# yixuan/LBFGSpp

Measured on AMD Instinct MI355X. Metric: L-BFGS iterations/sec at n=10^8, m=10; achieved HBM GB/s vs peak, higher is better.
Workload: dtype f64; 1 GPU; north-star: extended Rosenbrock n=100000000 m=10 f64 LineSearchMoreThuente, x0 from counter hash; n=100000000, m=10, history_full=True, fevals_total=111, apply_Hv_persistent_launches=82

## Files before the change

### include/lbfgsx.h

```cpp
#ifndef LBFGSX_H
#define LBFGSX_H

#include <stddef.h>
#include <stdint.h>

#ifdef __cplusplus
extern "C" {
#endif

typedef struct lbfgsx_ctx lbfgsx_ctx;

enum { LBFGSX_F64 = 0, LBFGSX_F32 = 1 };
enum { LBFGSX_OBJ_NONE = -1, LBFGSX_OBJ_DIAG_QUAD = 0, LBFGSX_OBJ_EXT_ROSENBROCK = 1,
       LBFGSX_OBJ_BOUND = 64  };
enum
{
    LBFGSX_OK = 0,
    LBFGSX_E_INVALID = -1,
    LBFGSX_E_LOGIC = -2,
    LBFGSX_E_RUNTIME = -3,
    LBFGSX_E_HIP = -4,
    LBFGSX_E_NOGPU = -5,
    LBFGSX_E_USER = -6
};
// ... 49 lines not shown
int lbfgsx_trial(lbfgsx_ctx* c, int objective, double step, double* fx, double* dg);
int lbfgsx_trial_point(lbfgsx_ctx* c, double step);
int lbfgsx_trial_dg(lbfgsx_ctx* c, double* dg);
int lbfgsx_ls_keep_trial_as_lo(lbfgsx_ctx* c);
int lbfgsx_ls_end(lbfgsx_ctx* c, int use_lo);
int lbfgsx_post_linesearch(lbfgsx_ctx* c, double* gnorm2, double* xnorm2, double* sy, double* yy);
int lbfgsx_commit_correction(lbfgsx_ctx* c);
int lbfgsx_post_linesearch_spec(lbfgsx_ctx* c, double a, double* gnorm2, double* xnorm2, double* sy, double* yy);
int lbfgsx_spec_counts(const lbfgsx_ctx* c, int64_t out[3]);
int lbfgsx_ls_post_in_trial(lbfgsx_ctx* c, double a);
int lbfgsx_post_in_trial_counts(const lbfgsx_ctx* c, int64_t out[4]);
int lbfgsx_last_in_trial_request(lbfgsx_ctx* c, int on);
int lbfgsx_apply_Hv_pending(lbfgsx_ctx* c, int v_which, double a, double* dg, int* pending);
int lbfgsx_trial_first(lbfgsx_ctx* c, int objective, double step, double* fx, double* dg, double* dg_init);
int lbfgsx_last_in_trial_counts(const lbfgsx_ctx* c, int64_t out[4]);
typedef struct lbfgsx_objective lbfgsx_objective;
int lbfgsx_objective_compile(lbfgsx_objective** out, int dtype, int K, const char* body, char* log, size_t log_len);
void lbfgsx_objective_destroy(lbfgsx_objective* obj);
long long lbfgsx_objective_source(int dtype, int K, const char* body, char* out, size_t len);
int lbfgsx_objective_info(const lbfgsx_objective* obj, long long out[8]);
int lbfgsx_objective_K(const lbfgsx_objective* obj);
int lbfgsx_objective_dtype(const lbfgsx_objective* obj);
int lbfgsx_objective_bind(lbfgsx_ctx* c, const lbfgsx_objective* obj, const void* const p[4], const double cs[8], int* id);
int lbfgsx_objective_upload(lbfgsx_ctx* c, int slot, const void* host, void** dev);
int lbfgsx_objective_bound(const lbfgsx_ctx* c, const void* p[4]);
enum { LBFGSX_FORM_TERM = 0, LBFGSX_FORM_CHAIN = 1, LBFGSX_FORM_GRID = 2, LBFGSX_FORM_GRAPH = 3, LBFGSX_FORM_MESH = 4, LBFGSX_FORM_LINEAR = 5,
       LBFGSX_FORM_LINEAR_MULTI = 6, LBFGSX_FORM_DENSE = 7, LBFGSX_FORM_LINEAR_GRAPH = 8, LBFGSX_FORM_VOLUME = 9,
       LBFGSX_FORM_GRID_PERIODIC = 10, LBFGSX_FORM_VOLUME_PERIODIC = 11, LBFGSX_FORM_GRID_FIELD = 12,
       LBFGSX_FORM_GRID_STENCIL = 13 };
int lbfgsx_objective_compile_chain(lbfgsx_objective** out, int dtype, int K, const char* body, char* log, size_t log_len);
// ... 282 lines not shown
```

### lbfgspp_amd/_lib.py

```python
import ctypes as C
import os

HERE = os.path.dirname(os.path.abspath(__file__))

F64, F32 = 0, 1
OBJ_DIAG_QUAD, OBJ_EXT_ROSENBROCK = 0, 1
OBJ_BOUND = 64
LS_NOCEDAL_WRIGHT, LS_MORE_THUENTE, LS_BACKTRACKING, LS_BRACKETING = 0, 1, 2, 3
ALGO_LBFGS, ALGO_LBFGSB = 0, 1
RECURSION_VECTOR, RECURSION_GRAM_SPACE, RECURSION_GRAM_SPACE_F32H = 0, 1, 2
FLAG_BOUNDED = 1
(VEC_X, VEC_G, VEC_XP, VEC_GP, VEC_D, VEC_XT, VEC_GT, VEC_A, VEC_B, VEC_LB, VEC_UB, VEC_XCP) = range(12)
E_INVALID, E_LOGIC, E_RUNTIME, E_HIP, E_NOGPU, E_USER = -1, -2, -3, -4, -5, -6


class Params(C.Structure):
    _fields_ = [("m", C.c_int), ("epsilon", C.c_double), ("epsilon_rel", C.c_double), ("past", C.c_int),
                ("delta", C.c_double), ("max_iterations", C.c_int), ("linesearch", C.c_int),
                ("max_linesearch", C.c_int), ("min_step", C.c_double), ("max_step", C.c_double),
                ("ftol", C.c_double), ("wolfe", C.c_double), ("max_submin", C.c_int)]


class Result(C.Structure):
    _fields_ = [("niter", C.c_int), ("nfev", C.c_int), ("fx", C.c_double), ("gnorm", C.c_double),
# ... 86 lines not shown
    sig(core, "lbfgsx_timing_enable", i32, vp, i32)
    sig(core, "lbfgsx_timing_read", i32, vp, pd, C.POINTER(i64), pd, C.POINTER(i64))
    sig(core, "lbfgsx_stream_probe", i32, vp, i32, pd, pd)
    sig(core, "lbfgsx_selftest_reduce", i32, vp, i32, i32, i32, pd)
    sig(core, "lbfgsx_post_linesearch_spec", i32, vp, dbl, pd, pd, pd, pd)
    sig(core, "lbfgsx_rccl_allgather_records", i32, C.POINTER(i32), i32, vp, i64, i64, C.POINTER(vp))
    sig(core, "lbfgsx_device_download", i32, i32, vp, i64, vp)
    sig(core, "lbfgsx_device_free", None, i32, vp)
    sig(core, "lbfgsx_spec_counts", i32, vp, C.POINTER(i64 * 3))
    sig(core, "lbfgsx_ls_post_in_trial", i32, vp, dbl)
    sig(core, "lbfgsx_post_in_trial_counts", i32, vp, C.POINTER(i64 * 4))
    sig(core, "lbfgsx_last_in_trial_request", i32, vp, i32)
    sig(core, "lbfgsx_apply_Hv_pending", i32, vp, i32, dbl, pd, C.POINTER(i32))
    sig(core, "lbfgsx_trial_first", i32, vp, i32, dbl, pd, pd, pd)
    sig(core, "lbfgsx_last_in_trial_counts", i32, vp, C.POINTER(i64 * 4))
    sig(core, "lbfgsx_counters", i32, C.POINTER(i64 * 3), i32)
    sig(core, "lbfgsx_counters_ex", i32, C.POINTER(i64 * 8), i32)
    sig(core, "lbfgsx_poll_counts", i32, vp, C.POINTER(i64 * 2))
    sig(core, "lbfgsx_poll_counts_ex", i32, vp, C.POINTER(i64 * 4))
    sig(core, "lbfgsx_b_compact_vec_counts", i32, C.POINTER(i64 * 4), i32)
    sig(core, "lbfgsx_b_reserve", i32, vp)
    sig(core, "lbfgsx_device", i32, vp)
    sig(core, "lbfgsx_persist_counts", i32, vp, C.POINTER(i64 * 4))
    sig(core, "lbfgsx_debug_persist_fault", i32, vp)

    sig(sol, "lbfgsx_solver_create", i32, C.POINTER(vp), i32, i32, i32, C.POINTER(Params), i32)
    sig(sol, "lbfgsx_solver_create_error", C.c_char_p)
    sig(sol, "lbfgsx_solver_destroy", None, vp)
    sig(sol, "lbfgsx_solver_prepare", i32, vp, i64)
    sig(sol, "lbfgsx_solver_ctx", vp, vp)
# ... 186 lines not shown
```

### lbfgspp_amd/csrc/ctx.hpp

```cpp
#pragma once
#include <hip/hip_runtime.h>
#include <stdint.h>

#include <atomic>
#include <chrono>
#include <string>
#include <vector>

#include "../../include/lbfgsx.h"
#include "last_step.hpp"
#include "reduce.cuh"

struct lbfgsx_ctx;
namespace lbfgsx {

void set_error(const std::string& msg);

#define LBFGSX_HIP(expr)                                                                      \
    do                                                                                        \
    {                                                                                         \
        hipError_t e_ = (expr);                                                               \
        if (e_ != hipSuccess)                                                                 \
        {                                                                                     \
            lbfgsx::set_error(std::string(#expr) + ": " + hipGetErrorString(e_) + " [" + __FILE__ + ":" + std::to_string(__LINE__) + "]");            \
            return LBFGSX_E_HIP;                                                              \
// ... 177 lines not shown
    int spec_cur = 0;
    double spec_a = 0.0, spec_dg = 0.0;
    int64_t spec_launches = 0, spec_used = 0, spec_rejected = 0;
    bool post_in_trial = true;
    bool pt_armed = false;
    double pt_a = 0.0;
    int ls_trials = 0;
    bool ls_first_ok = false;
    bool pt_valid = false;
    int pt_buf = -1, pt_xp = -1;
    double pt_r[4] = {0, 0, 0, 0};
    int64_t pt_issued = 0, pt_accepted = 0;
    int64_t from_g_launches = 0;
    lbfgsx::LastStep last;
    bool pt_builtin = false;

    const struct lbfgsx_objective* term = nullptr;
    void* term_fn[8] = {nullptr, nullptr, nullptr, nullptr, nullptr, nullptr, nullptr, nullptr};
    const void* term_p[4] = {nullptr, nullptr, nullptr, nullptr};
    double term_c[8] = {0, 0, 0, 0, 0, 0, 0, 0};
    int term_np = 0;
    int term_form = 0;
    int64_t term_rows = 0, term_cols = 0;
    int64_t term_slabs = 0;
    int term_periodic = 0;
    void* term_own[4] = {nullptr, nullptr, nullptr, nullptr};
    int64_t term_own_count[4] = {0, 0, 0, 0};
    int64_t graph_E = 0;
    void* graph_off = nullptr;
    void* graph_inc = nullptr;
// ... 121 lines not shown
```

### lbfgspp_amd/csrc/jit_objective.hip

```cpp
#include <dlfcn.h>
#include <hip/hiprtc.h>

#include <chrono>
#include <cstdio>
#include <cstdlib>
#include <cstring>
#include <map>
#include <memory>
#include <mutex>
#include <string>
#include <vector>

#include "form_table.hpp"
#include "launch_args.hpp"

namespace {

using lbfgsx::kFormRows;

struct BodyDesc
{
    const char* comment;
    const char* signature;
    const char* line;
// ... 824 lines not shown

int lbfgsx_objective_upload(lbfgsx_ctx* c, int slot, const void* host, void** dev)
{
    return lbfgsx_objective_upload_count(c, slot, host, c ? c->n : 0, dev);
}

}

namespace {

int objective_bind(lbfgsx_ctx* c, const lbfgsx_objective* obj, int64_t rows, int64_t cols, const void* const p[4],
                   const double cs[8], int* id, int64_t slabs = 0, int periodic = 0)
{
    c->st_valid = false;
    c->spec_valid = false;
    if (!obj)
    {
        c->term = nullptr;
        c->term_np = 0;
        c->term_form = LBFGSX_FORM_TERM;
        c->term_slabs = c->term_rows = c->term_cols = 0;
        c->term_periodic = 0;
        if (c->graph_inc || c->lin.colptr || c->dense.w)
        {
            lbfgsx::DeviceGuard dev_guard_(c->device);
            (void) lbfgsx::stream_sync(c->stream);
            lbfgsx::graph_topology_free(c);
        }
        if (id)
            *id = LBFGSX_OBJ_NONE;
// ... 69 lines not shown

bool handle_is(const lbfgsx_objective* obj, int form)
{
    const lbfgsx::FormRow& f = kFormRows[form];
    if (obj->code->form == form)
        return true;
    lbfgsx::set_error(std::string("lbfgsx_objective_bind") + f.suffix + ": the handle is a " + kFormRows[obj->code->form].name +
                      ", not a " + f.name + " (lbfgsx_objective_compile" + f.suffix + ")");
    return false;
}

int bind_begin(lbfgsx_ctx* c, const lbfgsx_objective* obj, int form)
{
    c->st_valid = false;
    c->spec_valid = false;
    c->term = nullptr;
    c->term_np = 0;
    c->term_form = LBFGSX_FORM_TERM;
    if (!handle_is(obj, form))
        return LBFGSX_E_INVALID;
    if (obj->code->dtype != c->dtype)
    {
        lbfgsx::set_error("lbfgsx_objective_bind: the objective was compiled for the other dtype");
        return LBFGSX_E_INVALID;
    }
    return LBFGSX_OK;
}

int bind_end(lbfgsx_ctx* c, const lbfgsx_objective* obj, const void* const p[4], const double cs[8], int* id)
{
// ... 396 lines not shown
```

### lbfgspp_amd/csrc/last_step.hpp

```cpp
#pragma once
#include <cstdint>

namespace lbfgsx {

struct LastStep
{
    bool enabled = true;
    bool requested = false;
    bool pending = false;
    bool taken = false;
    int cn = 0;
    int col = 0;
    int g = 0;
    bool owed = false;
    int64_t deferred = 0, fused = 0, settled = 0;

    bool want(bool post_form_on, bool builtin_objective, bool first_trial_accepted, int pairs, bool sharded,
              bool vector_recursion) const
    {
        return enabled && requested && post_form_on && builtin_objective && first_trial_accepted && pairs >= 1 && !sharded &&
               vector_recursion;
    }
    void defer(int pairs, int newest_col, int g_buf)
    {
        pending = true;
        taken = owed = false;
        cn = pairs;
        col = newest_col;
        g = g_buf;
        deferred++;
    }
    bool fusable(bool post_form, bool builtin_objective, bool caller_reads_dg, int xp_buf) const
    {
        return pending && !taken && post_form && builtin_objective && caller_reads_dg && xp_buf == g;
    }
    void fuse()
    {
        taken = true;
        fused++;
    }
    template <class F>
    int settle(F&& launch)
    {
        if (!pending)
            return 0;
// ... 19 lines not shown
```

### lbfgspp_amd/csrc/lbfgs_kernels.cuh

```cuda
#pragma once
#include "reduce.cuh"

namespace lbfgsx {

enum { OBJ_DIAG_QUAD = 0, OBJ_EXT_ROSENBROCK = 1 };

template <class T>
struct ObjQuad
{
    const T* a;
    const T* b;
    template <class A>
    __device__ __forceinline__ void pack(int64_t vi, const Pack<T>& x, Pack<T>& g, A& fx) const
    {
        const Pack<T> pa = ldv(a, vi), pb = ldv(b, vi);
#pragma unroll
        for (int k = 0; k < Vec16<T>::W; k++)
        {
            const T r = pa.e[k] * x.e[k] - pb.e[k];
            g.e[k] = pa.e[k] * r;
            fx.add(r * r);
        }
    }
    __device__ __forceinline__ T finish(T sum) const { return T(0.5) * sum; }
// ... 86 lines not shown
    T* dot0;
};

template <class T>
struct TrialLast
{
    const T* snew;
    const T* num;
    const T* num2;
    const T* den;
    T* dot0_keep;
    T* dg_slot;
    T* dout;
};

template <class T, class OBJ, bool POST, bool LAST = false>
__device__ __forceinline__ void trial_pass(const T* __restrict__ xp, const T* __restrict__ d, T step, T* __restrict__ x,
                                           T* __restrict__ g, int64_t n, const OBJ& obj, const RedWs& ws,
                                           T* __restrict__ out, int rev, const TrialPost<T>& tp,
                                           const TrialLast<T>& tl = TrialLast<T>())
{
    typedef typename AccOf<T>::type A;
    constexpr int W = Vec16<T>::W;
    constexpr int U = 4;
    constexpr bool SETTLE = LAST && !POST;
    constexpr int NRED = POST ? (LAST ? 8 : 7) : 2;
    A acc[NRED];
    T coef = T(0);
    if (LAST)
        coef = *tl.num / *tl.den - *tl.num2 / *tl.den;
    const int64_t nv = n / W;
    const int64_t tile = int64_t(kBlock) * U;
    const int64_t top = ((nv + tile - 1) / tile - 1) * tile;
    for (int64_t t0 = int64_t(blockIdx.x) * tile; t0 < nv; t0 += int64_t(gridDim.x) * tile)
    {
        const int64_t base = (rev ? top - t0 : t0) + threadIdx.x;
        Pack<T> pxp[U], pd[U], pgp[POST ? U : 1], psn[LAST ? U : 1];
#pragma unroll
        for (int u = 0; u < U; u++)
            if (base + u * kBlock < nv)
            {
// ... 5 lines not shown
                    pgp[POST ? u : 0] = ldv(tp.gp, base + u * kBlock);
            }
#pragma unroll
        for (int u = 0; u < U; u++)
        {
            const int64_t vi = base + u * kBlock;
            if (vi < nv)
            {
                Pack<T> px, pg;
                if (LAST)
                {
#pragma unroll
                    for (int k = 0; k < W; k++)
                    {
                        pd[u].e[k] = pd[u].e[k] + coef * psn[LAST ? u : 0].e[k];
                        if (POST)
                            acc[POST && LAST ? 7 : 0].add_prod(pgp[POST ? u : 0].e[k], pd[u].e[k]);
                    }
                    if (SETTLE)
                        stv(tl.dout, vi, pd[u]);
                }
#pragma unroll
                for (int k = 0; k < W; k++)
                    px.e[k] = pxp[u].e[k] + step * pd[u].e[k];
                obj.pack(vi, px, pg, acc[0]);
                stv(x, vi, px);
                stv(g, vi, pg);
#pragma unroll
                for (int k = 0; k < W; k++)
                    acc[1].add_prod(pg.e[k], pd[u].e[k]);
                if (POST)
                {
// ... 14 lines not shown
                    stv(tp.y, vi, py);
                }
            }
        }
    }
    if (blockIdx.x == 0 && threadIdx.x == 0)
    {
        auto dir = [&](int64_t i) { return LAST ? d[i] + coef * tl.snew[i] : d[i]; };
        for (int64_t i = nv * W; i < n; i++)
            x[i] = xp[i] + step * dir(i);
        for (int64_t i = nv * W; i < n; i++)
        {
            const T di = dir(i);
            obj.tail(i, n, x, g, acc[0]);
            acc[1].add_prod(g[i], di);
            if (POST && LAST)
                acc[POST && LAST ? 7 : 0].add_prod(tp.gp[i], di);
            if (SETTLE)
                tl.dout[i] = di;
        }
        if (POST)
            for (int64_t i = nv * W; i < n; i++)
            {
                const T si = x[i] - xp[i], yi = g[i] - tp.gp[i], q0 = tp.a * g[i];
                tp.s[i] = si;
                tp.y[i] = yi;
                acc[POST ? 2 : 0].add_prod(g[i], g[i]);
                acc[POST ? 3 : 0].add_prod(x[i], x[i]);
                acc[POST ? 4 : 0].add_prod(si, yi);
                acc[POST ? 5 : 0].add_prod(yi, yi);
                acc[POST ? 6 : 0].add_prod(si, q0);
            }
    }
    if (grid_reduce<NRED>(acc, ws) && threadIdx.x == 0)
    {
        out[0] = obj.finish(T(acc[0].value()));
        out[1] = T(acc[1].value());
        if (POST)
        {
            const T sy = T(acc[POST ? 4 : 0].value()), yy = T(acc[POST ? 5 : 0].value());
            out[2] = T(acc[POST ? 2 : 0].value());
            out[3] = T(acc[POST ? 3 : 0].value());
            out[4] = sy;
            out[5] = yy;
            if (LAST)
            {
                const T dgd = T(acc[LAST ? 7 : 0].value());
                out[6] = dgd;
                *tl.dg_slot = dgd;
                *tl.dot0_keep = *tl.num;
            }
            *tp.ys_slot = sy;
            *tp.theta_slot = yy / sy;
            *tp.dot0 = T(acc[POST ? 6 : 0].value());
        }
        ws_signal(ws);
    }
}

template <class T, class OBJ>
__global__ void __launch_bounds__(kBlock) k_trial(const T* __restrict__ xp, const T* __restrict__ d, T step,
                                                  T* __restrict__ x, T* __restrict__ g, int64_t n, OBJ obj,
// ... 10 lines not shown
}
template <class T, class OBJ>
__global__ void __launch_bounds__(kBlock, 4) k_trial_last(const T* __restrict__ xp, const T* __restrict__ q, T step,
                                                       T* __restrict__ x, T* __restrict__ g, int64_t n, OBJ obj,
                                                       RedWs ws, T* __restrict__ out, int rev, TrialPost<T> tp,
                                                       TrialLast<T> tl)
{
    trial_pass<T, OBJ, true, true>(xp, q, step, x, g, n, obj, ws, out, rev, tp, tl);
}
template <class T, class OBJ>
__global__ void __launch_bounds__(kBlock) k_trial_settle(const T* __restrict__ xp, const T* q, T step, T* __restrict__ x,
                                                         T* __restrict__ g, int64_t n, OBJ obj, RedWs ws,
                                                         T* __restrict__ out, int rev, TrialLast<T> tl)
{
    trial_pass<T, OBJ, false, true>(xp, q, step, x, g, n, obj, ws, out, rev, TrialPost<T>(), tl);
}

template <class T>
__global__ void __launch_bounds__(kBlock) k_axpy_point(const T* __restrict__ xp, const T* __restrict__ d, T step,
                                                       T* __restrict__ x, int64_t n)
{
    constexpr int W = Vec16<T>::W;
    const int64_t nv = n / W;
    const int64_t stride = int64_t(gridDim.x) * kBlock;
    for (int64_t vi = int64_t(blockIdx.x) * kBlock + threadIdx.x; vi < nv; vi += stride)
    {
        const Pack<T> pxp = ldv(xp, vi), pd = ldv(d, vi);
        Pack<T> px;
#pragma unroll
        for (int k = 0; k < W; k++)
// ... 968 lines not shown
```

### lbfgspp_amd/csrc/lbfgsx.hip

```cpp
#include <dlfcn.h>

#include <algorithm>
#include <atomic>
#include <cmath>
#include <chrono>
#include <string>
#include <vector>
#include <utility>
#include <cstdio>
#include <cstdlib>
#include <cstring>
#include <limits>
#include <mutex>

#include "ctx.hpp"
#include "lbfgs_kernels.cuh"
#include "launch_args.hpp"

namespace lbfgsx {

static std::atomic<int> g_live[64];
Counters& counters()
{
    static Counters g;
// ... 365 lines not shown
        if (n < min_n)
            c->persist = false;
    }
    if (const char* e = getenv("LBFGSX_PERSIST"))
        c->persist = atoi(e) != 0 && c->persist;
    if (const char* e = getenv("LBFGSX_MEET"))
        c->meet_all = std::strcmp(e, "last") != 0;
    if (const char* e = getenv("LBFGSX_PERSIST_POLL"))
        c->fast_persist_out = atoi(e) != 0;
    if (const char* e = getenv("LBFGSX_FUSE_POST"))
        c->fuse_post = atoi(e) != 0;
    if (const char* e = getenv("LBFGSX_POST_IN_TRIAL"))
        c->post_in_trial = atoi(e) != 0;
    if (const char* e = getenv("LBFGSX_LAST_IN_TRIAL"))
        c->last.enabled = atoi(e) != 0;
    {
        int occ = 0;
        hipDeviceProp_t prop;
        LBFGSX_HIP(hipGetDeviceProperties(&prop, device));
        if (dtype == LBFGSX_F64)
            (void) hipOccupancyMaxActiveBlocksPerMultiprocessor(&occ, k_twoloop_persist<double, true, true>, kHvThreads, 0);
        else
            (void) hipOccupancyMaxActiveBlocksPerMultiprocessor(&occ, k_twoloop_persist<float, true, true>, kHvThreads, 0);
        c->persist_grid = occ * prop.multiProcessorCount;
        c->gen_words = 16 + size_t(10) * size_t(c->persist_grid) * 4;
        LBFGSX_HIP(hipMalloc(reinterpret_cast<void**>(&c->gen_dev), c->gen_words * sizeof(unsigned)));
        LBFGSX_HIP(hipMemset(c->gen_dev, 0, c->gen_words * sizeof(unsigned)));
    }
    const size_t vbytes = size_t(c->ld) * c->esz;
    for (int k = 0; k < 3; k++)
// ... 138 lines not shown
}

int64_t lbfgsx_n(const lbfgsx_ctx* c) { return c->n; }
void* lbfgsx_vec(lbfgsx_ctx* c, int which)
{
    if (which == LBFGSX_VEC_D && lbfgsx::last_settle(c))
        return nullptr;
    return vec_ptr(c, which);
}

int lbfgsx_upload(lbfgsx_ctx* c, int which, const void* host)
{
    lbfgsx::DeviceGuard dev_guard_(c->device);
    c->vec_writes++;
    c->spec_valid = false;
    LBFGSX_SETTLE(c);
    void* p = vec_ptr(c, which);
    if (!p || !host)
    {
        set_error("lbfgsx_upload: unknown vector or null host pointer");
        return LBFGSX_E_INVALID;
    }
    LBFGSX_HIP(lbfgsx::copy_async(p, host, size_t(c->n) * c->esz, hipMemcpyHostToDevice, c->stream));
    LBFGSX_HIP(lbfgsx::stream_sync(c->stream));
    return LBFGSX_OK;
}

int lbfgsx_download(lbfgsx_ctx* c, int which, void* host)
{
    lbfgsx::DeviceGuard dev_guard_(c->device);
    LBFGSX_SETTLE(c);
    void* p = vec_ptr(c, which);
    if (!p || !host)
    {
        set_error("lbfgsx_download: unknown vector or null host pointer");
        return LBFGSX_E_INVALID;
    }
    LBFGSX_HIP(lbfgsx::copy_async(host, p, size_t(c->n) * c->esz, hipMemcpyDeviceToHost, c->stream));
    LBFGSX_HIP(lbfgsx::stream_sync(c->stream));
    return LBFGSX_OK;
}

int lbfgsx_gather(lbfgsx_ctx* c, int which, int64_t stride, double* host)
{
    lbfgsx::DeviceGuard dev_guard_(c->device);
    LBFGSX_SETTLE(c);
// ... 23 lines not shown
{
    if (!c || offset < 0 || n_global < offset + c->n)
    {
        set_error("lbfgsx_set_shard: need 0 <= offset and offset + n <= n_global");
        return LBFGSX_E_INVALID;
    }
    c->shard_off = offset;
    c->n_global = n_global;
    return LBFGSX_OK;
}

int lbfgsx_gen_diag_quad(lbfgsx_ctx* c, double kappa, uint64_t seed)
{
    lbfgsx::DeviceGuard dev_guard_(c->device);
    c->spec_valid = false;
    DISPATCH_T(c, { LBFGSX_LAUNCH(k_gen_quad<T>, dim3(2048), dim3(256), 0, c->stream, P<T>(c->a), P<T>(c->b),
                                       c->n, kappa, seed, c->shard_off, c->n_global); });
    LBFGSX_HIP(hipGetLastError());
    return LBFGSX_OK;
}

int lbfgsx_gen_rosen_x0(lbfgsx_ctx* c, uint64_t seed)
{
    lbfgsx::DeviceGuard dev_guard_(c->device);
    c->vec_writes++;
    c->spec_valid = false;
    DISPATCH_T(c, { LBFGSX_LAUNCH(k_gen_rosen<T>, dim3(2048), dim3(256), 0, c->stream, P<T>(c->xb[c->cur]),
                                       c->n, seed, c->shard_off); });
    LBFGSX_HIP(hipGetLastError());
    return LBFGSX_OK;
}

int lbfgsx_fill(lbfgsx_ctx* c, int which, double value)
{
    lbfgsx::DeviceGuard dev_guard_(c->device);
    c->vec_writes++;
    c->spec_valid = false;
    LBFGSX_SETTLE(c);
    void* p = vec_ptr(c, which);
    if (!p)
    {
        set_error("lbfgsx_fill: unknown vector");
        return LBFGSX_E_INVALID;
    }
    DISPATCH_T(c, { LBFGSX_LAUNCH(k_fill<T>, dim3(2048), dim3(256), 0, c->stream, P<T>(p), c->n, T(value)); });
    LBFGSX_HIP(hipGetLastError());
    return LBFGSX_OK;
}

int lbfgsx_bfgs_reset(lbfgsx_ctx* c)
{
    lbfgsx::DeviceGuard dev_guard_(c->device);
    c->theta = 1.0;
    c->ncorr = 0;
    c->ptr = c->m;
    c->pending = false;
    c->spec_valid = false;
    c->pt_valid = c->pt_armed = c->ls_first_ok = false;
    c->last.drop();
    c->ls_trials = 0;
    c->tl_step = 0;
    for (int j = 0; j < c->m; j++)
        c->phys[size_t(j)] = j;
    c->phys_version++;
    c->spare = c->m;
    DISPATCH_T(c, {
        T one = T(1);
        LBFGSX_HIP(lbfgsx::copy_async(P<T>(c->sc) + c->sl.one(), &one, sizeof(T), hipMemcpyHostToDevice, c->stream));
        LBFGSX_HIP(lbfgsx::stream_sync(c->stream));
    });
    return LBFGSX_OK;
}

// ... 399 lines not shown
        const T* g = P<T>(c->gb[c->cur]);
        LBFGSX_LAUNCH((k_dot<T>), dim3(grid), dim3(kBlock), 0, c->stream, g, g, P<T>(c->xb[c->cur]), c->n, c->ws,
                           c->out_slot<T>());
        int rc = fetch_scalars<T>(c, c->sl.out(0), 2, r);
        if (rc)
            return rc;
    });
    if (gnorm2) *gnorm2 = r[0];
    if (xnorm2) *xnorm2 = r[1];
    return LBFGSX_OK;
}

int lbfgsx_ls_begin(lbfgsx_ctx* c)
{
    c->st_valid = false;
    c->pt_valid = c->pt_armed = false;
    c->ls_trials = 0;
    c->xp = c->cur;
    c->lo = c->xp;
    c->trial = (c->xp + 1) % 3;
    return LBFGSX_OK;
}

}
template <class T, class OBJ>
static int trial_t(lbfgsx_ctx* c, OBJ obj, T step, double* out2)
{
    const lbfgsx::TrialLaunch<T> a = lbfgsx::trial_launch<T>(c, step, sizeof(OBJ) >= 2 * sizeof(void*) ? 2 : 0);
    LBFGSX_LAUNCH((k_trial<T, OBJ>), dim3(a.grid), dim3(kBlock), 0, c->stream, a.xp, a.d, a.step, a.x, a.g, a.n, obj, a.ws,
                       a.out, a.rev);
    LBFGSX_HIP(hipGetLastError());
    return fetch_scalars<T>(c, c->sl.out(0), 2, out2);
// ... 1 lines not shown
template <class T>
static lbfgsx::TrialPost<T> trial_post_args(lbfgsx_ctx* c)
{
    T* sc = P<T>(c->sc);
    return {P<T>(c->gb[c->xp]), P<T>(c->col(c->S, c->spare)), P<T>(c->col(c->Y, c->spare)), T(c->pt_a),
            sc + c->sl.ys(c->spare), sc + c->sl.theta(c->spare), sc + c->sl.dot(0)};
}
static void trial_post_done(lbfgsx_ctx* c, const double* out6)
{
    c->pending = false;
    c->pt_valid = true;
    c->pt_buf = c->trial;
    c->pt_xp = c->xp;
    for (int i = 0; i < 4; i++)
        c->pt_r[i] = out6[2 + i];
    c->pt_issued++;
}
template <class T, class OBJ>
static int trial_post_t(lbfgsx_ctx* c, OBJ obj, T step, double* out2)
{
    const lbfgsx::TrialLaunch<T> a = lbfgsx::trial_launch<T>(c, step, sizeof(OBJ) >= 2 * sizeof(void*) ? 2 : 0);
    const lbfgsx::TrialPost<T> tp = trial_post_args<T>(c);
    LBFGSX_LAUNCH((k_trial_post<T, OBJ>), dim3(a.grid), dim3(kBlock), 0, c->stream, a.xp, a.d, a.step, a.x, a.g, a.n, obj,
                       a.ws, a.out, a.rev, tp);
    LBFGSX_HIP(hipGetLastError());
    double r[6];
    const int rc = fetch_scalars<T>(c, c->sl.out(0), 6, r);
    if (rc)
        return rc;
    out2[0] = r[0];
    out2[1] = r[1];
// ... 44 lines not shown
    const lbfgsx::TrialLaunch<T> a = lbfgsx::trial_launch<T>(c, step, (sizeof(OBJ) >= 2 * sizeof(void*) ? 2 : 0) + 2);
    T* sc = P<T>(c->sc);
    const lbfgsx::TrialLast<T> tl = {static_cast<const T*>(c->col(c->S, ls.col)), sc + c->sl.dot(2 * c->m + 1),
                                     sc + c->sl.dot(2 * ls.cn - 1), sc + c->sl.ys(ls.col), nullptr, nullptr, P<T>(c->d)};
    EventPair ev;
    int rc = last_time_begin(c, ev);
    if (rc)
        return rc;
    LBFGSX_LAUNCH((k_trial_settle<T, OBJ>), dim3(a.grid), dim3(kBlock), 0, c->stream, a.xp, a.d, a.step, a.x, a.g, a.n, obj,
                       a.ws, a.out, a.rev, tl);
    LBFGSX_HIP(hipGetLastError());
    if ((rc = last_time_end(c, ev)))
        return rc;
    (void) c->last.settle([](const lbfgsx::LastStep&) { return 0; });
    return fetch_scalars<T>(c, c->sl.out(0), 2, out2);
}
template <class T>
static int trial_post_term_t(lbfgsx_ctx* c, T step, double* out2)
{
    lbfgsx::TrialLaunch<T> a = lbfgsx::trial_launch<T>(c, step, c->term_np);
    lbfgsx::BoundArgs<T> obj(c);
    lbfgsx::TrialPost<T> tp = trial_post_args<T>(c);
    void* params[] = {&a.xp, &a.d, &a.step, &a.x, &a.g, &a.n, obj.ptr, &a.ws, &a.out, &a.rev, &tp};
    int rc = lbfgsx::jit_launch(c, lbfgsx::JIT_K_TRIAL_POST, a.grid, params);
    if (rc)
        return rc;
    double r[6];
    rc = fetch_scalars<T>(c, c->sl.out(0), 6, r);
    if (rc)
        return rc;
// ... 47 lines not shown
        DISPATCH_T(c, { same = same && T(step) == T(c->st_step); });
        if (same)
        {
            c->st_hits++;
            c->ls_trials++;
            c->tl_step++;
            if (fx) *fx = c->st_f;
            if (dg) *dg = c->st_dg;
            return LBFGSX_OK;
        }
        c->st_cooldown = 4;
    }
    const bool post = c->pt_armed && c->ls_trials == 0 &&
                      (objective == LBFGSX_OBJ_DIAG_QUAD || objective == LBFGSX_OBJ_EXT_ROSENBROCK ||
                       (lbfgsx::term_bound(c, objective) && c->term_fn[lbfgsx::JIT_K_TRIAL_POST] != nullptr));
    c->ls_trials++;
    c->pt_valid = false;
    DISPATCH_T(c, {
        if (objective == LBFGSX_OBJ_DIAG_QUAD)
            rc = last          ? trial_last_t<T>(c, ObjQuad<T>{P<T>(c->a), P<T>(c->b)}, T(step), r)
                 : settle_here ? trial_settle_t<T>(c, ObjQuad<T>{P<T>(c->a), P<T>(c->b)}, T(step), r)
                 : post        ? trial_post_t<T>(c, ObjQuad<T>{P<T>(c->a), P<T>(c->b)}, T(step), r)
                               : trial_t<T>(c, ObjQuad<T>{P<T>(c->a), P<T>(c->b)}, T(step), r);
        else if (objective == LBFGSX_OBJ_EXT_ROSENBROCK)
            rc = last          ? trial_last_t<T>(c, ObjRosen<T>{}, T(step), r)
                 : settle_here ? trial_settle_t<T>(c, ObjRosen<T>{}, T(step), r)
                 : post        ? trial_post_t<T>(c, ObjRosen<T>{}, T(step), r)
                               : trial_t<T>(c, ObjRosen<T>{}, T(step), r);
        else if (lbfgsx::term_bound(c, objective))
            rc = post ? trial_post_term_t<T>(c, T(step), r) : trial_term_t<T>(c, T(step), r);
        else
            set_error("lbfgsx_trial: unknown objective");
        if (!rc && owed)
            rc = fetch_scalars<T>(c, c->sl.dot(2 * last_cn), 1, dg_init);
    });
    if (rc)
        return rc;
    if (fx) *fx = r[0];
    if (dg) *dg = r[1];
    if (last) *dg_init = r[2];
    return LBFGSX_OK;
}
// ... 32 lines not shown
{
    if (c->lo == c->xp)
    {
        c->lo = c->trial;
        c->trial = third_point(c->xp, c->lo);
    }
    else
        std::swap(c->lo, c->trial);
    return LBFGSX_OK;
}

int lbfgsx_ls_end(lbfgsx_ctx* c, int use_lo)
{
    c->cur = use_lo ? c->lo : c->trial;
    c->ls_first_ok = !use_lo && c->ls_trials == 1;
    return LBFGSX_OK;
}

int lbfgsx_post_linesearch(lbfgsx_ctx* c, double* gnorm2, double* xnorm2, double* sy, double* yy)
{
    lbfgsx::DeviceGuard dev_guard_(c->device);
    c->spec_valid = false;
    c->pt_valid = false;
    if (c->gs_f32h)
    {
        set_error("lbfgsx_post_linesearch: this context keeps its history in f32 for the Gram-space recursion (lbfgsx_gs_set_history_dtype)");
        return LBFGSX_E_LOGIC;
    }
    const int grid = c->grid_for(c->n);
    double r[4];
// ... 39 lines not shown
        pa.pcol[i] = 0;
    {
        int j = loc;
        for (int i = 0; i < cn; i++)
        {
            pa.pcol[i] = (j == loc) ? c->spare : c->phys[size_t(j)];
            j = (j + m - 1) % m;
        }
    }
    pa.gen_base = c->gen_count;
    pa.zigzag = 1;
    pa.first_rev = c->tl_step;
    pa.pub_first = 1;
    pa.ld = c->ld;
    pa.from_g = from_g ? 1 : 0;
    const bool defer = from_g && !c->bstate &&
                       c->last.want(c->post_in_trial, c->pt_builtin, c->ls_first_ok, cn, c->shard_off != 0 || c->n_global != c->n,
                                    !c->gs_f32h);
    pa.defer_last = defer ? 1 : 0;
    c->gen_count += unsigned(2 * cn + 1);
    c->tl_step += unsigned(2 * cn + 1 - pa.defer_last);
    T* sc = P<T>(c->sc);
    PostFuse<T> pf;
    pf.x = P<T>(c->xb[c->cur]);
    pf.xp = P<T>(c->xb[c->xp]);
    pf.gp = P<T>(c->gb[c->xp]);
    pf.s = P<T>(c->col(c->S, c->spare));
    pf.y = P<T>(c->col(c->Y, c->spare));
    pf.out = c->out_slot<T>();
    pf.ys_slot = sc + c->sl.ys(c->spare);
    pf.theta_slot = sc + c->sl.theta(c->spare);
    pf.eps = std::numeric_limits<T>::epsilon();
    pf.verdict = reinterpret_cast<int*>(c->gen_dev + 2);
// ... 72 lines not shown
        LBFGSX_HIP(hipMemsetAsync(c->ws.ticket, 0, sizeof(unsigned), c->stream));
        c->gen_count = 0;
        persist_timed_out(c);
        if (c->timing && !c->ev_hv.empty())
        {
            (void) hipEventDestroy(c->ev_hv.back().a);
            (void) hipEventDestroy(c->ev_hv.back().b);
            c->ev_hv.pop_back();
            c->persist_steps_timed -= 2 * cn + 1;
            c->fused_timed -= fused;
        }
        return 1;
    }
    c->persist_launches++;
    c->spec_launches++;
    c->from_g_launches += from_g ? 1 : 0;
    c->persist_backoff = 8;
    if (hflags[1] == 1)
    {
        c->spec_valid = true;
        c->spec_version = c->phys_version + 1;
        c->spec_cur = c->cur;
        c->spec_a = double(a);
        c->spec_dg = dgv;
        if (defer)
        {
            c->spec_dg = std::numeric_limits<double>::quiet_NaN();
            c->last.defer(cn, pa.pcol[0], c->cur);
        }
    }
    else
    {
        c->spec_rejected++;
        if (c->timing && !c->ev_hv.empty())
        {
            (void) hipEventDestroy(c->ev_hv.back().a);
            (void) hipEventDestroy(c->ev_hv.back().b);
            c->ev_hv.pop_back();
            c->persist_steps_timed -= 2 * cn + 1;
            c->fused_timed -= fused;
        }
    }
    return LBFGSX_OK;
}
extern "C" {

int lbfgsx_post_linesearch_spec(lbfgsx_ctx* c, double a, double* gnorm2, double* xnorm2, double* sy, double* yy)
{
    lbfgsx::DeviceGuard dev_guard_(c->device);
    if (c->gs_f32h)
        return lbfgsx_post_linesearch(c, gnorm2, xnorm2, sy, yy);
    double r[4];
    int rc = 1;
    c->spec_valid = false;
    if (c->pt_valid && c->cur == c->pt_buf && c->xp == c->pt_xp)
    {
        c->pt_valid = false;
        c->pt_accepted++;
        for (int i = 0; i < 4; i++)
            r[i] = c->pt_r[i];
        c->pend_sy = r[2];
        c->pend_yy = r[3];
        c->pending = true;
        bool usable = false;
        DISPATCH_T(c, { usable = a == c->pt_a && T(r[2]) > std::numeric_limits<T>::epsilon() * T(r[3]); });
        if (usable)
        {
            DISPATCH_T(c, { rc = post_spec_t<T>(c, T(a), r, true); });
            if (rc != LBFGSX_OK && rc != 1)
                return rc;
        }
        if (gnorm2) *gnorm2 = r[0];
        if (xnorm2) *xnorm2 = r[1];
// ... 10 lines not shown
    c->pend_sy = r[2];
    c->pend_yy = r[3];
    c->pending = true;
    if (gnorm2) *gnorm2 = r[0];
    if (xnorm2) *xnorm2 = r[1];
    if (sy) *sy = r[2];
    if (yy) *yy = r[3];
    return LBFGSX_OK;
}

int lbfgsx_ls_post_in_trial(lbfgsx_ctx* c, double a)
{
    if (!c)
        return LBFGSX_E_INVALID;
    c->pt_a = a;
    c->pt_armed = c->post_in_trial && c->ls_first_ok && c->ncorr > 0 && !c->gs_f32h && c->ls_trials == 0 &&
                  c->shard_off == 0 && c->n_global == c->n;
    return LBFGSX_OK;
}

int lbfgsx_post_in_trial_counts(const lbfgsx_ctx* c, int64_t out[4])
{
    if (!c || !out)
        return LBFGSX_E_INVALID;
    out[0] = c->pt_issued;
    out[1] = c->pt_accepted;
    out[2] = c->from_g_launches;
    out[3] = c->post_in_trial ? 1 : 0;
    return LBFGSX_OK;
}

int lbfgsx_last_in_trial_request(lbfgsx_ctx* c, int on)
// ... 337 lines not shown
```

Before: 93.63 iterations/s.

## Add evidence-based trial policy to arm fused post pass on first and second trials

Adds a sliding-window TrialPolicy that records recent line-search outcomes. It arms the fused trial-plus-post-linesearch pass on the first trial when most recent searches ended there, and on the second trial (including a new settle+post kernel) when second trials usually end the search. The goal is to avoid separate post-linesearch reduction passes over the 10^8-element vectors. The cost is extra speculative reduction work when a prediction is wrong, plus added bookkeeping and invalidation logic. It also restricts settle on download to the direction vector only.

```diff
diff --git a/include/lbfgsx.h b/include/lbfgsx.h
--- a/include/lbfgsx.h
+++ b/include/lbfgsx.h
@@ -87,6 +87,7 @@
 int lbfgsx_apply_Hv_pending(lbfgsx_ctx* c, int v_which, double a, double* dg, int* pending);
 int lbfgsx_trial_first(lbfgsx_ctx* c, int objective, double step, double* fx, double* dg, double* dg_init);
 int lbfgsx_last_in_trial_counts(const lbfgsx_ctx* c, int64_t out[4]);
+int lbfgsx_trial_policy_counts(const lbfgsx_ctx* c, int64_t out[8]);
 typedef struct lbfgsx_objective lbfgsx_objective;
 int lbfgsx_objective_compile(lbfgsx_objective** out, int dtype, int K, const char* body, char* log, size_t log_len);
 void lbfgsx_objective_destroy(lbfgsx_objective* obj);
diff --git a/lbfgspp_amd/_lib.py b/lbfgspp_amd/_lib.py
--- a/lbfgspp_amd/_lib.py
+++ b/lbfgspp_amd/_lib.py
@@ -124,6 +124,7 @@
     sig(core, "lbfgsx_apply_Hv_pending", i32, vp, i32, dbl, pd, C.POINTER(i32))
     sig(core, "lbfgsx_trial_first", i32, vp, i32, dbl, pd, pd, pd)
     sig(core, "lbfgsx_last_in_trial_counts", i32, vp, C.POINTER(i64 * 4))
+    sig(core, "lbfgsx_trial_policy_counts", i32, vp, C.POINTER(i64 * 8))
     sig(core, "lbfgsx_counters", i32, C.POINTER(i64 * 3), i32)
     sig(core, "lbfgsx_counters_ex", i32, C.POINTER(i64 * 8), i32)
     sig(core, "lbfgsx_poll_counts", i32, vp, C.POINTER(i64 * 2))
diff --git a/lbfgspp_amd/csrc/ctx.hpp b/lbfgspp_amd/csrc/ctx.hpp
--- a/lbfgspp_amd/csrc/ctx.hpp
+++ b/lbfgspp_amd/csrc/ctx.hpp
@@ -9,6 +9,7 @@
 
 #include "../../include/lbfgsx.h"
 #include "last_step.hpp"
+#include "trial_policy.hpp"
 #include "reduce.cuh"
 
 struct lbfgsx_ctx;
@@ -216,6 +217,11 @@
     int64_t from_g_launches = 0;
     lbfgsx::LastStep last;
     bool pt_builtin = false;
+    lbfgsx::TrialPolicy policy;
+    bool pt_armed2 = false;
+    bool pt_by_evidence = false;
+    int pt_trial = 0;
+    int policy_obj = -1;
 
     const struct lbfgsx_objective* term = nullptr;
     void* term_fn[8] = {nullptr, nullptr, nullptr, nullptr, nullptr, nullptr, nullptr, nullptr};
diff --git a/lbfgspp_amd/csrc/jit_objective.hip b/lbfgspp_amd/csrc/jit_objective.hip
--- a/lbfgspp_amd/csrc/jit_objective.hip
+++ b/lbfgspp_amd/csrc/jit_objective.hip
@@ -862,6 +862,7 @@
 {
     c->st_valid = false;
     c->spec_valid = false;
+    c->policy.clear();
     if (!obj)
     {
         c->term = nullptr;
@@ -961,6 +962,7 @@
 {
     c->st_valid = false;
     c->spec_valid = false;
+    c->policy.clear();
     c->term = nullptr;
     c->term_np = 0;
     c->term_form = LBFGSX_FORM_TERM;
diff --git a/lbfgspp_amd/csrc/last_step.hpp b/lbfgspp_amd/csrc/last_step.hpp
--- a/lbfgspp_amd/csrc/last_step.hpp
+++ b/lbfgspp_amd/csrc/last_step.hpp
@@ -15,20 +15,20 @@
     bool owed = false;
     int64_t deferred = 0, fused = 0, settled = 0;
 
-    bool want(bool post_form_on, bool builtin_objective, bool first_trial_accepted, int pairs, bool sharded,
+    bool want(bool post_form_on, bool builtin_objective, bool next_first_armed, int pairs, bool sharded,
               bool vector_recursion) const
     {
-        return enabled && requested && post_form_on && builtin_objective && first_trial_accepted && pairs >= 1 && !sharded &&
+        return enabled && requested && post_form_on && builtin_objective && next_first_armed && pairs >= 1 && !sharded &&
                vector_recursion;
     }
-    void defer(int pairs, int newest_col, int g_buf)
+    void defer(int pairs, int newest_col, int g_buf, bool behind_first_trial = true)
     {
         pending = true;
         taken = owed = false;
         cn = pairs;
         col = newest_col;
         g = g_buf;
-        deferred++;
+        deferred += behind_first_trial ? 1 : 0;
     }
     bool fusable(bool post_form, bool builtin_objective, bool caller_reads_dg, int xp_buf) const
     {
diff --git a/lbfgspp_amd/csrc/lbfgs_kernels.cuh b/lbfgspp_amd/csrc/lbfgs_kernels.cuh
--- a/lbfgspp_amd/csrc/lbfgs_kernels.cuh
+++ b/lbfgspp_amd/csrc/lbfgs_kernels.cuh
@@ -124,7 +124,7 @@
     T* dout;
 };
 
-template <class T, class OBJ, bool POST, bool LAST = false>
+template <class T, class OBJ, bool POST, bool LAST = false, bool SETTLE = LAST && !POST>
 __device__ __forceinline__ void trial_pass(const T* __restrict__ xp, const T* __restrict__ d, T step, T* __restrict__ x,
                                            T* __restrict__ g, int64_t n, const OBJ& obj, const RedWs& ws,
                                            T* __restrict__ out, int rev, const TrialPost<T>& tp,
@@ -133,8 +133,8 @@
     typedef typename AccOf<T>::type A;
     constexpr int W = Vec16<T>::W;
     constexpr int U = 4;
-    constexpr bool SETTLE = LAST && !POST;
-    constexpr int NRED = POST ? (LAST ? 8 : 7) : 2;
+    constexpr bool DGD = POST && LAST && !SETTLE;
+    constexpr int NRED = POST ? (DGD ? 8 : 7) : 2;
     A acc[NRED];
     T coef = T(0);
     if (LAST)
@@ -170,8 +170,8 @@
                     for (int k = 0; k < W; k++)
                     {
                         pd[u].e[k] = pd[u].e[k] + coef * psn[LAST ? u : 0].e[k];
-                        if (POST)
-                            acc[POST && LAST ? 7 : 0].add_prod(pgp[POST ? u : 0].e[k], pd[u].e[k]);
+                        if (DGD)
+                            acc[DGD ? 7 : 0].add_prod(pgp[POST ? u : 0].e[k], pd[u].e[k]);
                     }
                     if (SETTLE)
                         stv(tl.dout, vi, pd[u]);
@@ -216,8 +216,8 @@
             const T di = dir(i);
             obj.tail(i, n, x, g, acc[0]);
             acc[1].add_prod(g[i], di);
-            if (POST && LAST)
-                acc[POST && LAST ? 7 : 0].add_prod(tp.gp[i], di);
+            if (DGD)
+                acc[DGD ? 7 : 0].add_prod(tp.gp[i], di);
             if (SETTLE)
                 tl.dout[i] = di;
         }
@@ -245,9 +245,9 @@
             out[3] = T(acc[POST ? 3 : 0].value());
             out[4] = sy;
             out[5] = yy;
-            if (LAST)
-            {
-                const T dgd = T(acc[LAST ? 7 : 0].value());
+            if (DGD)
+            {
+                const T dgd = T(acc[DGD ? 7 : 0].value());
                 out[6] = dgd;
                 *tl.dg_slot = dgd;
                 *tl.dot0_keep = *tl.num;
@@ -288,6 +288,14 @@
                                                          T* __restrict__ out, int rev, TrialLast<T> tl)
 {
     trial_pass<T, OBJ, false, true>(xp, q, step, x, g, n, obj, ws, out, rev, TrialPost<T>(), tl);
+}
+template <class T, class OBJ>
+__global__ void __launch_bounds__(kBlock, 4) k_trial_settle_post(const T* __restrict__ xp, const T* q, T step,
+                                                                 T* __restrict__ x, T* __restrict__ g, int64_t n, OBJ obj,
+                                                                 RedWs ws, T* __restrict__ out, int rev, TrialPost<T> tp,
+                                                                 TrialLast<T> tl)
+{
+    trial_pass<T, OBJ, true, true, true>(xp, q, step, x, g, n, obj, ws, out, rev, tp, tl);
 }
 
 template <class T>
diff --git a/lbfgspp_amd/csrc/lbfgsx.hip b/lbfgspp_amd/csrc/lbfgsx.hip
--- a/lbfgspp_amd/csrc/lbfgsx.hip
+++ b/lbfgspp_amd/csrc/lbfgsx.hip
@@ -403,6 +403,8 @@
         c->post_in_trial = atoi(e) != 0;
     if (const char* e = getenv("LBFGSX_LAST_IN_TRIAL"))
         c->last.enabled = atoi(e) != 0;
+    if (const char* e = getenv("LBFGSX_TRIAL_EVIDENCE"))
+        c->policy.enabled = atoi(e) != 0;
     {
         int occ = 0;
         hipDeviceProp_t prop;
@@ -571,6 +573,9 @@
     lbfgsx::DeviceGuard dev_guard_(c->device);
     c->vec_writes++;
     c->spec_valid = false;
+    c->pt_valid = false;
+    if (which == LBFGSX_VEC_A || which == LBFGSX_VEC_B)
+        c->policy.clear();
     LBFGSX_SETTLE(c);
     void* p = vec_ptr(c, which);
     if (!p || !host)
@@ -586,7 +591,8 @@
 int lbfgsx_download(lbfgsx_ctx* c, int which, void* host)
 {
     lbfgsx::DeviceGuard dev_guard_(c->device);
-    LBFGSX_SETTLE(c);
+    if (which == LBFGSX_VEC_D)
+        LBFGSX_SETTLE(c);
     void* p = vec_ptr(c, which);
     if (!p || !host)
     {
@@ -640,6 +646,8 @@
 {
     lbfgsx::DeviceGuard dev_guard_(c->device);
     c->spec_valid = false;
+    c->pt_valid = false;
+    c->policy.clear();
     DISPATCH_T(c, { LBFGSX_LAUNCH(k_gen_quad<T>, dim3(2048), dim3(256), 0, c->stream, P<T>(c->a), P<T>(c->b),
                                        c->n, kappa, seed, c->shard_off, c->n_global); });
     LBFGSX_HIP(hipGetLastError());
@@ -651,6 +659,7 @@
     lbfgsx::DeviceGuard dev_guard_(c->device);
     c->vec_writes++;
     c->spec_valid = false;
+    c->pt_valid = false;
     DISPATCH_T(c, { LBFGSX_LAUNCH(k_gen_rosen<T>, dim3(2048), dim3(256), 0, c->stream, P<T>(c->xb[c->cur]),
                                        c->n, seed, c->shard_off); });
     LBFGSX_HIP(hipGetLastError());
@@ -662,6 +671,7 @@
     lbfgsx::DeviceGuard dev_guard_(c->device);
     c->vec_writes++;
     c->spec_valid = false;
+    c->pt_valid = false;
     LBFGSX_SETTLE(c);
     void* p = vec_ptr(c, which);
     if (!p)
@@ -682,7 +692,8 @@
     c->ptr = c->m;
     c->pending = false;
     c->spec_valid = false;
-    c->pt_valid = c->pt_armed = c->ls_first_ok = false;
+    c->pt_valid = c->pt_armed = c->pt_armed2 = c->pt_by_evidence = c->ls_first_ok = false;
+    c->policy.clear();
     c->last.drop();
     c->ls_trials = 0;
     c->tl_step = 0;
@@ -1112,8 +1123,9 @@
 int lbfgsx_ls_begin(lbfgsx_ctx* c)
 {
     c->st_valid = false;
-    c->pt_valid = c->pt_armed = false;
+    c->pt_valid = c->pt_armed = c->pt_armed2 = c->pt_by_evidence = false;
     c->ls_trials = 0;
+    c->policy.begin(c->ncorr > 0);
     c->xp = c->cur;
     c->lo = c->xp;
     c->trial = (c->xp + 1) % 3;
@@ -1145,7 +1157,14 @@
     c->pt_xp = c->xp;
     for (int i = 0; i < 4; i++)
         c->pt_r[i] = out6[2 + i];
-    c->pt_issued++;
+    c->pt_trial = c->ls_trials;
+    if (c->pt_trial == 1)
+    {
+        c->pt_issued++;
+        c->policy.first_by_evidence += c->pt_by_evidence ? 1 : 0;
+    }
+    else
+        c->policy.second_issued++;
 }
 template <class T, class OBJ>
 static int trial_post_t(lbfgsx_ctx* c, OBJ obj, T step, double* out2)
@@ -1220,6 +1239,40 @@
         return rc;
     (void) c->last.settle([](const lbfgsx::LastStep&) { return 0; });
     return fetch_scalars<T>(c, c->sl.out(0), 2, out2);
+}
+template <class T, class OBJ>
+static int trial_settle_post_t(lbfgsx_ctx* c, OBJ obj, T step, double* out2)
+{
+    const lbfgsx::LastStep& ls = c->last;
+    if (ls.col == c->spare)
+    {
+        set_error("lbfgsx_trial: the newest history column is the spare column");
+        return LBFGSX_E_LOGIC;
+    }
+    const lbfgsx::TrialLaunch<T> a = lbfgsx::trial_launch<T>(c, step, (sizeof(OBJ) >= 2 * sizeof(void*) ? 2 : 0) + 2);
+    const lbfgsx::TrialPost<T> tp = trial_post_args<T>(c);
+    T* sc = P<T>(c->sc);
+    const lbfgsx::TrialLast<T> tl = {static_cast<const T*>(c->col(c->S, ls.col)), sc + c->sl.dot(2 * c->m + 1),
+                                     sc + c->sl.dot(2 * ls.cn - 1), sc + c->sl.ys(ls.col), nullptr, nullptr, P<T>(c->d)};
+    EventPair ev;
+    int rc = last_time_begin(c, ev);
+    if (rc)
+        return rc;
+    LBFGSX_LAUNCH((k_trial_settle_post<T, OBJ>), dim3(a.grid), dim3(kBlock), 0, c->stream, a.xp, a.d, a.step, a.x, a.g, a.n,
+                       obj, a.ws, a.out, a.rev, tp, tl);
+    LBFGSX_HIP(hipGetLastError());
+    if ((rc = last_time_end(c, ev)))
+        return rc;
+    (void) c->last.settle([](const lbfgsx::LastStep&) { return 0; });
+    double r[6];
+    rc = fetch_scalars<T>(c, c->sl.out(0), 6, r);
+    if (rc)
+        return rc;
+    out2[0] = r[0];
+    out2[1] = r[1];
+    trial_post_done(c, r);
+    c->pt_builtin = true;
+    return LBFGSX_OK;
 }
 template <class T>
 static int trial_post_term_t(lbfgsx_ctx* c, T step, double* out2)
@@ -1297,18 +1350,26 @@
     const bool post = c->pt_armed && c->ls_trials == 0 &&
                       (objective == LBFGSX_OBJ_DIAG_QUAD || objective == LBFGSX_OBJ_EXT_ROSENBROCK ||
                        (lbfgsx::term_bound(c, objective) && c->term_fn[lbfgsx::JIT_K_TRIAL_POST] != nullptr));
+    const bool post2 = c->pt_armed2 && c->ls_trials == 1 && builtin;
+    if (objective != c->policy_obj)
+    {
+        c->policy.clear();
+        c->policy_obj = objective;
+    }
     c->ls_trials++;
     c->pt_valid = false;
     DISPATCH_T(c, {
         if (objective == LBFGSX_OBJ_DIAG_QUAD)
             rc = last          ? trial_last_t<T>(c, ObjQuad<T>{P<T>(c->a), P<T>(c->b)}, T(step), r)
-                 : settle_here ? trial_settle_t<T>(c, ObjQuad<T>{P<T>(c->a), P<T>(c->b)}, T(step), r)
-                 : post        ? trial_post_t<T>(c, ObjQuad<T>{P<T>(c->a), P<T>(c->b)}, T(step), r)
+                 : settle_here ? (post2 ? trial_settle_post_t<T>(c, ObjQuad<T>{P<T>(c->a), P<T>(c->b)}, T(step), r)
+                                        : trial_settle_t<T>(c, ObjQuad<T>{P<T>(c->a), P<T>(c->b)}, T(step), r))
+                 : post || post2 ? trial_post_t<T>(c, ObjQuad<T>{P<T>(c->a), P<T>(c->b)}, T(step), r)
                                : trial_t<T>(c, ObjQuad<T>{P<T>(c->a), P<T>(c->b)}, T(step), r);
         else if (objective == LBFGSX_OBJ_EXT_ROSENBROCK)
             rc = last          ? trial_last_t<T>(c, ObjRosen<T>{}, T(step), r)
-                 : settle_here ? trial_settle_t<T>(c, ObjRosen<T>{}, T(step), r)
-                 : post        ? trial_post_t<T>(c, ObjRosen<T>{}, T(step), r)
+                 : settle_here ? (post2 ? trial_settle_post_t<T>(c, ObjRosen<T>{}, T(step), r)
+                                        : trial_settle_t<T>(c, ObjRosen<T>{}, T(step), r))
+                 : post || post2 ? trial_post_t<T>(c, ObjRosen<T>{}, T(step), r)
                                : trial_t<T>(c, ObjRosen<T>{}, T(step), r);
         else if (lbfgsx::term_bound(c, objective))
             rc = post ? trial_post_term_t<T>(c, T(step), r) : trial_term_t<T>(c, T(step), r);
@@ -1371,6 +1432,9 @@
 {
     c->cur = use_lo ? c->lo : c->trial;
     c->ls_first_ok = !use_lo && c->ls_trials == 1;
+    c->policy.end(c->ls_trials, use_lo != 0);
+    if (use_lo && c->pt_trial != 1)
+        c->pt_valid = false;
     return LBFGSX_OK;
 }
 
@@ -1440,9 +1504,10 @@
     pa.pub_first = 1;
     pa.ld = c->ld;
     pa.from_g = from_g ? 1 : 0;
+    const bool behind2 = from_g && c->pt_trial == 2;
     const bool defer = from_g && !c->bstate &&
-                       c->last.want(c->post_in_trial, c->pt_builtin, c->ls_first_ok, cn, c->shard_off != 0 || c->n_global != c->n,
-                                    !c->gs_f32h);
+                       c->last.want(c->post_in_trial, c->pt_builtin, c->policy.arm_first(c->ls_first_ok), cn,
+                                    c->shard_off != 0 || c->n_global != c->n, !c->gs_f32h);
     pa.defer_last = defer ? 1 : 0;
     c->gen_count += unsigned(2 * cn + 1);
     c->tl_step += unsigned(2 * cn + 1 - pa.defer_last);
@@ -1545,7 +1610,8 @@
     }
     c->persist_launches++;
     c->spec_launches++;
-    c->from_g_launches += from_g ? 1 : 0;
+    c->from_g_launches += from_g && !behind2 ? 1 : 0;
+    c->policy.second_from_g += behind2 ? 1 : 0;
     c->persist_backoff = 8;
     if (hflags[1] == 1)
     {
@@ -1557,7 +1623,8 @@
         if (defer)
         {
             c->spec_dg = std::numeric_limits<double>::quiet_NaN();
-            c->last.defer(cn, pa.pcol[0], c->cur);
+            c->last.defer(cn, pa.pcol[0], c->cur, !behind2);
+            c->policy.second_deferred += behind2 ? 1 : 0;
         }
     }
     else
@@ -1584,10 +1651,16 @@
     double r[4];
     int rc = 1;
     c->spec_valid = false;
-    if (c->pt_valid && c->cur == c->pt_buf && c->xp == c->pt_xp)
+    if (c->pt_valid && c->cur == c->pt_buf && c->xp == c->pt_xp && c->ls_trials == c->pt_trial)
     {
         c->pt_valid = false;
-        c->pt_accepted++;
+        if (c->pt_trial == 1)
+        {
+            c->pt_accepted++;
+            c->policy.first_by_evidence_accepted += c->pt_by_evidence ? 1 : 0;
+        }
+        else
+            c->policy.second_accepted++;
         for (int i = 0; i < 4; i++)
             r[i] = c->pt_r[i];
         c->pend_sy = r[2];
@@ -1628,8 +1701,27 @@
     if (!c)
         return LBFGSX_E_INVALID;
     c->pt_a = a;
-    c->pt_armed = c->post_in_trial && c->ls_first_ok && c->ncorr > 0 && !c->gs_f32h && c->ls_trials == 0 &&
-                  c->shard_off == 0 && c->n_global == c->n;
+    const bool can = c->post_in_trial && c->ncorr > 0 && !c->gs_f32h && c->ls_trials == 0 && c->shard_off == 0 &&
+                     c->n_global == c->n;
+    c->pt_armed = can && c->policy.arm_first(c->ls_first_ok);
+    c->pt_by_evidence = c->pt_armed && !c->ls_first_ok;
+    c->pt_armed2 = can && c->policy.arm_second();
+    return LBFGSX_OK;
+}
+
+int lbfgsx_trial_policy_counts(const lbfgsx_ctx* c, int64_t out[8])
+{
+    if (!c || !out)
+        return LBFGSX_E_INVALID;
+    const lbfgsx::TrialPolicy& p = c->policy;
+    out[0] = p.held;
+    out[1] = p.first_by_evidence;
+    out[2] = p.first_by_evidence_accepted;
+    out[3] = p.second_issued;
+    out[4] = p.second_accepted;
+    out[5] = p.second_from_g;
+    out[6] = p.second_deferred;
+    out[7] = p.enabled ? 1 : 0;
     return LBFGSX_OK;
 }
 
diff --git a/lbfgspp_amd/csrc/trial_policy.hpp b/lbfgspp_amd/csrc/trial_policy.hpp
--- /dev/null
+++ b/lbfgspp_amd/csrc/trial_policy.hpp
@@ -0,0 +1,72 @@
+#pragma once
+#include <cstdint>
+
+namespace lbfgsx {
+
+struct TrialPolicy
+{
+    static constexpr int kWindow = 16;
+    enum : uint8_t { FIRST_OK = 1, HAD_SECOND = 2, ENDED_AT_SECOND = 4 };
+
+    bool enabled = true;
+    uint8_t ring[kWindow] = {};
+    int head = 0;
+    int held = 0;
+    bool open = false;
+    bool sample = false;
+    int64_t first_by_evidence = 0, first_by_evidence_accepted = 0;
+    int64_t second_issued = 0, second_accepted = 0;
+    int64_t second_from_g = 0, second_deferred = 0;
+
+    void clear()
+    {
+        head = held = 0;
+        open = sample = false;
+    }
+    void begin(bool history_non_empty)
+    {
+        open = true;
+        sample = history_non_empty;
+    }
+    void end(int trials, bool at_kept_point)
+    {
+        const bool take = open && sample && trials >= 1;
+        open = false;
+        if (!take)
+            return;
+        uint8_t e = 0;
+        if (trials == 1 && !at_kept_point)
+            e |= FIRST_OK;
+        if (trials >= 2)
+            e |= HAD_SECOND;
+        if (trials == 2 && !at_kept_point)
+            e |= ENDED_AT_SECOND;
+        ring[head] = e;
+        head = (head + 1) % kWindow;
+        if (held < kWindow)
+            held++;
+    }
+    int count(uint8_t bit) const
+    {
+        int k = 0;
+        for (int i = 0; i < held; i++)
+            k += (ring[i] & bit) ? 1 : 0;
+        return k;
+    }
+    bool evidence() const { return enabled && held == kWindow; }
+    bool arm_first(bool prev_first_ok) const
+    {
+        if (!evidence())
+            return prev_first_ok;
+        return 2 * count(FIRST_OK) >= kWindow;
+    }
+    bool arm_second() const
+    {
+        if (!evidence())
+            return false;
+        const int reached = count(HAD_SECOND);
+        return reached >= 1 && 2 * count(ENDED_AT_SECOND) >= reached;
+    }
+};
+
+}
```

Measured after the change: 94.57 iterations/s, median of 6. 1.0% higher.
